# lpylpy0514/VitTracker

Measured on AMD Instinct MI355X. Metric: track() frames/sec per GPU, vit_48_h32, 128px search / 64px template, higher is better.
Workload: dtype f32

## Files before the change

vittracker_amd/csrc/vittrack.hip:

```cpp
#include "../../include/vittrack.h"

#include <hip/hip_runtime.h>

#include <algorithm>
#include <array>
#include <cmath>
#include <cstdio>
#include <cstdlib>
#include <cstring>
#include <map>
#include <mutex>
#include <string>
#include <utility>
#include <vector>

#include "vb_api.h"
#include "vt_blocks.h"
#include "vt_blocks_tile.h"
#include "vt_head.h"
#ifndef VT_SEQ3_MAXP
#define VT_SEQ3_MAXP 2
#endif
#include "vt_head3.h"
#include "vt_generic.h"
// ... 133 lines not shown
    VbModel* vb = nullptr;
    bool generic = false;
    vtg::Dims gd{48, 1, 32};
    DevBuf g_stem_w[4], g_stem_b[4];
    DevBuf g_blocks;
    DevBuf g_head;
    DevBuf g_a, g_b;
    DevBuf g_qkv, g_ao, g_hid, g_x;
    vt_config cfg{};
    Switches sw;
    int len_z = 0, len_x = 0, L = 0, F = 0, Fz = 0;
    bool weights_loaded = false;
    DevBuf stem_w[4], stem_b[4];
    DevBuf stem_w3b;
    DevBuf stem_w4b;
    DevBuf stem_w2k;
    DevBuf stem_w1u;
    std::vector<double> stem_w1_f64, stem_b1_f64;
    float norm_mean[3] = {0.485f, 0.456f, 0.406f}, norm_std[3] = {0.229f, 0.224f, 0.225f};
    DevBuf pos_z, pos_x;
    DevBuf blocks;
    DevBuf blocks3;
    DevBuf head;
    DevBuf head3;
    DevBuf window;
    DevBuf act_x, act_z;
    DevBuf tokens, feat;
    DevBuf tokens_c;
    DevBuf tile_q, tile_k, tile_v, tile_x;
    DevBuf head_m1;
    int head_m1_frames = 0;
// ... 378 lines not shown
    if (m->generic) {
        if (xu8 && zmode != 1) return fail(VT_ERR_STATE, "this stem form has no uint8-patch variant");
        return gen_stem(m, z, x, B, st, tokens, zmode, xu8);
    }
    StemForm f;
    if (int rc = select_stem(m, form_b(m, B), zmode, xu8, &f)) return rc;
    const float* const w1 = xu8 ? m->stem_w1u.p : m->stem_w[0].p;
    const float* const b1 = xu8 ? m->stem_w1u.p + vts::W1U_BIAS : m->stem_b[0].p;
    const int Tx = m->cfg.search_size, Tz = m->cfg.template_size;
    float* const act_x = m->act_x.p + f0 * (size_t)(Tx / 4) * (Tx / 4) * 12;
    float* const act_z = m->act_z.p + f0 * (size_t)(Tz / 4) * (Tz / 4) * 12;
    const int skip_a = m->sw.skip_stem_a;
#ifndef VT_F16
    if (f.stream) {
        hipLaunchKernelGGL(f.stream->k, dim3(B), dim3(f.stream->block), f.stream->lds, st, z, x, w1, b1, m->stem_b[1].p, m->stem_w[2].p, m->stem_b[2].p,
                           m->stem_w[3].p, m->stem_b[3].p, m->pos_z.p, m->pos_x.p, tokens, m->L, m->len_z, m->stem_w2k.p);
        HIP_TRY(hipGetLastError());
        return VT_OK;
    }
#endif
    if (f.fused) {
        hipLaunchKernelGGL(f.fused->k, dim3(B), dim3(f.fused->block), f.fused->lds, st, z, x, w1, b1, m->stem_w[1].p, m->stem_b[1].p, m->stem_w[2].p,
                           m->stem_b[2].p, m->stem_w[3].p, m->stem_b[3].p, m->pos_z.p, m->pos_x.p, tokens, m->L, m->len_z, skip_a, m->dbg_stamps,
                           m->stem_w2k.p, m->stem_w3b.p, m->stem_w4b.p);
        HIP_TRY(hipGetLastError());
        return VT_OK;
    }
    vts::CropA ax{x, act_x, Tx, f.px.r2, zmode == 2 ? 0 : (Tx / 4) / f.px.r2}, az{z, act_z, Tz, f.pz.r2, zmode == 1 ? 0 : (Tz / 4) / f.pz.r2};
    if (f.pipe)
        hipLaunchKernelGGL(f.pipe->k, dim3(B), dim3(f.pipe->block), f.pipe->lds, st, z, x, w1, b1, m->stem_w[1].p, m->stem_b[1].p, act_z, act_x, skip_a,
                           m->dbg_stamps, m->stem_w2k.p);
    else if (f.a2)
        hipLaunchKernelGGL(vts::stem_a2_kernel, dim3(B * ax.bands), dim3(256), f.lds_a, st, ax, az, m->stem_w[0].p, m->stem_b[0].p, m->stem_w[1].p,
                           m->stem_b[1].p, skip_a);
    else
        hipLaunchKernelGGL(f.a->k, dim3(B * (ax.bands + az.bands)), dim3(f.a->block), f.lds_a, st, ax, az, w1, b1, m->stem_w[1].p, m->stem_b[1].p, skip_a);
    HIP_TRY(hipGetLastError());
    vts::CropB bx{act_x, m->pos_x.p, Tx / 4, f.px.r4, zmode == 2 ? 0 : (Tx / 16) / f.px.r4, m->len_z};
    vts::CropB bz{act_z, m->pos_z.p, Tz / 4, f.pz.r4, zmode == 1 ? 0 : (Tz / 16) / f.pz.r4, 0};
    hipLaunchKernelGGL(f.b->k, dim3(B * (bx.bands + bz.bands)), dim3(f.b->block), f.lds_b, st, bx, bz, m->stem_w[2].p, m->stem_b[2].p, m->stem_w[3].p,
                       m->stem_b[3].p, tokens, m->L, m->sw.skip_stem_b);
    HIP_TRY(hipGetLastError());
    return VT_OK;
}

struct BlocksForm {
// ... 548 lines not shown
    }
    if (rc) {
        vt_destroy(m);
        return rc;
    }
    *out = m;
    return VT_OK;
}

void vt_destroy(vt_model* m) {
    if (!m) return;
    for (vt_graph* g : m->graphs) g->owner = nullptr;
    m->graphs.clear();
    if (m->vb) vb::destroy(m->vb);
    for (int i = 0; i < 4; ++i) { m->stem_w[i].release(); m->stem_b[i].release(); }
    m->stem_w2k.release();
    m->stem_w1u.release();
    m->stem_w3b.release();
    m->stem_w4b.release();
    m->act_x.release(); m->act_z.release();
    DevBuf* all[] = {&m->pos_z, &m->pos_x, &m->blocks, &m->blocks3, &m->head, &m->head3, &m->window, &m->tokens, &m->feat, &m->zcache, &m->zstage, &m->imsizes, &m->vlscr, &m->tokens_c,
                     &m->tile_q, &m->tile_k, &m->tile_v, &m->tile_x, &m->head_m1,
                     &m->score, &m->size, &m->offset, &m->pred, &m->hann, &m->conf};
    for (DevBuf* d : all) d->release();
    for (int i = 0; i < 4; ++i) { m->g_stem_w[i].release(); m->g_stem_b[i].release(); }
    DevBuf* gen[] = {&m->g_blocks, &m->g_head, &m->g_a, &m->g_b, &m->g_qkv, &m->g_ao, &m->g_hid, &m->g_x};
    for (DevBuf* d : gen) d->release();
    if (m->cap_stream) (void)hipStreamDestroy(m->cap_stream);
    for (int i = 0; i < 3; ++i) {
        if (m->side_stream[i]) (void)hipStreamDestroy(m->side_stream[i]);
        if (m->join_ev[i]) (void)hipEventDestroy(m->join_ev[i]);
// ... 492 lines not shown
```

vittracker_amd/csrc/vt_conv.h:

```cpp
#pragma once
#include "vt_common.h"

namespace vtc {

template <int NQ>
__device__ __forceinline__ void decode_quad(int Q, int& tap, int& icq) {
    constexpr int NQT = 9 * NQ;
    Q = Q < NQT ? Q : NQT - 1;
    tap = Q / NQ;
    icq = Q - tap * NQ;
}

template <int NOT, int MAXC, int NCH>
__device__ __forceinline__ void load_weights(const float* __restrict__ wimg, int c0, int n, int lane,
                                             opnd (&a)[MAXC][NOT]) {
#pragma unroll
    for (int k = 0; k < MAXC; ++k)
        if (k < n)
#pragma unroll
            for (int ot = 0; ot < NOT; ++ot) a[k][ot] = *reinterpret_cast<const opnd*>(wimg + ((size_t)(ot * NCH + c0 + k) * 64 + lane) * 4);
    __builtin_amdgcn_sched_barrier(0);
}
template <int NOT, int MAXC, int NCH>
__device__ __forceinline__ void load_weights_f4(const float* __restrict__ wimg, int c0, int n, int lane,
// ... 54 lines not shown
                                                f4 (&acc)[NPT][NOT]) {
    constexpr int FULL = NCH / MAXC, REM = NCH % MAXC;
#pragma unroll
    for (int p = 0; p < FULL; ++p) {
        opnd a[MAXC][NOT];
        load_weights<NOT, MAXC, NCH>(wimg, p * MAXC, MAXC, lane, a);
        mma_pass<NOT, NPT, MAXC, MAXC>(in_map, base, a, p * MAXC, off, acc);
    }
    if constexpr (REM > 0) {
        opnd a[MAXC][NOT];
        load_weights<NOT, MAXC, NCH>(wimg, FULL * MAXC, REM, lane, a);
        mma_pass<NOT, NPT, MAXC, REM>(in_map, base, a, FULL * MAXC, off, acc);
    }
}

}
```

vittracker_amd/csrc/vt_head3.h:

```cpp
#pragma once
#include "vt_bf3.h"
#include "vt_head.h"

#ifndef VT_F16
#ifndef VT_SEQ3_C2_MAXP
#define VT_SEQ3_C2_MAXP 5
#endif
#ifndef VT_SEQ3_C2_ACT
#define VT_SEQ3_C2_ACT 8
#endif
#ifndef VT_H3_SKIP
#define VT_H3_SKIP 0
#endif
namespace vth3 {

using vth::C;
using vth::W1;
using vth::nchunks;
using vth::ntiles;
using vt3::bf16x8;
using vt3::u32x2;
using vt3::u32x4;
using vt3::split3;
using vt3::join3;
// ... 155 lines not shown
                    acc = __builtin_amdgcn_mfma_f32_16x16x32_bf16(__builtin_bit_cast(bf16x8, ww[wp]), __builtin_bit_cast(bf16x8, x[xp]), acc, 0, 0, 0);
                };
                if (!(VT_H3_SKIP & 2)) { mm(2, 0); mm(0, 2); mm(1, 1); mm(1, 0); mm(0, 1); mm(0, 0); }
            }
            if (p == NSP - 1 && 4 * q < COUT) {
                f4 v = acc;
                v.x = fmaxf(v.x, 0.f); v.y = fmaxf(v.y, 0.f); v.z = fmaxf(v.z, 0.f); v.w = fmaxf(v.w, 0.f);
                out_map[q * G::NPIX + centre] = v;
            }
            pipe.park(g + 1);
            __syncthreads();
        }
    }
};

template <int AB>
__device__ __forceinline__ f4 mfma4x4_bcast(float a, float b, f4 c) { return __builtin_amdgcn_mfma_f32_4x4x1f32(a, b, c, 4, AB, 0); }
__device__ __forceinline__ f4 mfma4x4_bcast(float a, float b, f4 c, int ab) {
    switch (ab) {
        case 0: return mfma4x4_bcast<0>(a, b, c);   case 1: return mfma4x4_bcast<1>(a, b, c);
        case 2: return mfma4x4_bcast<2>(a, b, c);   case 3: return mfma4x4_bcast<3>(a, b, c);
        case 4: return mfma4x4_bcast<4>(a, b, c);   case 5: return mfma4x4_bcast<5>(a, b, c);
        case 6: return mfma4x4_bcast<6>(a, b, c);   case 7: return mfma4x4_bcast<7>(a, b, c);
        case 8: return mfma4x4_bcast<8>(a, b, c);   case 9: return mfma4x4_bcast<9>(a, b, c);
        case 10: return mfma4x4_bcast<10>(a, b, c); case 11: return mfma4x4_bcast<11>(a, b, c);
        case 12: return mfma4x4_bcast<12>(a, b, c); case 13: return mfma4x4_bcast<13>(a, b, c);
        case 14: return mfma4x4_bcast<14>(a, b, c); default: return mfma4x4_bcast<15>(a, b, c);
    }
}
constexpr int quad_nkr(int nq) { return (9 * nq * 4 + 15) / 16; }
template <int NQ, int PLANE, typename Off>
__device__ __forceinline__ void quad_taps(const f4* in0, Off off, const float (&wr)[quad_nkr(NQ)], f4 (&acc)[4]) {
    f4 bv[2][NQ];
    auto fetch = [&](int tap, f4 (&bd)[NQ]) {
        const int o = off(tap);
#pragma unroll
        for (int icq = 0; icq < NQ; ++icq) bd[icq] = in0[icq * PLANE + o];
        __builtin_amdgcn_sched_barrier(0);
    };
    fetch(0, bv[0]);
#pragma unroll
    for (int tap = 0; tap < 9; ++tap) {
        if (tap + 1 < 9) fetch(tap + 1, bv[(tap + 1) & 1]);
#pragma unroll
// ... 519 lines not shown
```

vittracker_amd/csrc/vt_stem.h:

```cpp
#pragma once
#include <type_traits>

#include "vt_common.h"
#include "vt_conv.h"

namespace vts {

typedef __attribute__((address_space(4))) const float* sptr;
__device__ __forceinline__ sptr opaque(const float* p) {
    unsigned long long v = reinterpret_cast<unsigned long long>(p);
    asm volatile("" : "+s"(v));
    return (sptr)v;
}

constexpr int round16(int v) { return (v + 15) & ~15; }
template <int NQ>
__device__ __forceinline__ int s2_chunk_off(int c, int q, int npix_in, int pitch_in, int half_in) {
    int tap, icq;
    vtc::decode_quad<NQ>(4 * c + q, tap, icq);
    const int dy = tap / 3, dx = tap - 3 * dy;
    return icq * npix_in + dy * pitch_in + (dx == 1 ? 0 : (dx == 0 ? half_in : half_in + 1));
}

__device__ __forceinline__ int ilog2(int v) { return 31 - __clz(v); }
// ... 71 lines not shown
}
template <bool ZERO_TOP, typename Band>
__device__ __forceinline__ void ring_edges(f4* ring, const f4* other_ring, int pair, const Band& J, bool halo) {
    const int nrow = 2 * J.R2 + 1;
    if (pair < 2 * nrow) {
        const int plane = pair >= nrow ? 1 : 0;
        ring[plane * J.npix1 + (pair - plane * nrow) * J.PITCH + J.HALF] = splat4(0.f);
    }
    if ((ZERO_TOP || halo) && pair >= 128 && pair < 128 + 2 * J.PITCH) {
        const int e = pair - 128, plane = e >= J.PITCH ? 1 : 0, col = e - plane * J.PITCH;
        ring[plane * J.npix1 + col] = halo ? other_ring[plane * J.npix1 + 2 * J.R2 * J.PITCH + col] : splat4(0.f);
    }
}

#ifndef VT_F16
typedef float f16v __attribute__((ext_vector_type(16)));
template <typename Band>
__device__ __forceinline__ f16v l2_tile4(const f4* ring, const Band& J, const f4* cw2, const float* cb2, int gw, int q, int px) {
    const int op = 16 * (4 * gw + q) + px, yy = op >> J.lgW2, xx = op & ((1 << J.lgW2) - 1);
    const f4* src = ring + 2 * yy * J.PITCH + xx;
    const f4* wk = cw2 + px;
    const f4 bv2 = ld4(cb2 + 4 * q);
    f16v acc = {bv2.x, bv2.y, bv2.z, bv2.w, bv2.x, bv2.y, bv2.z, bv2.w, bv2.x, bv2.y, bv2.z, bv2.w, bv2.x, bv2.y, bv2.z, bv2.w};
    auto tapoff = [&](int tap) {
        const int dy = tap / 3, dx = tap - 3 * dy;
        return dy * J.PITCH + (dx == 1 ? 0 : (dx == 0 ? J.HALF : J.HALF + 1));
    };
    f4 a0 = src[tapoff(0)], a1 = src[J.npix1 + tapoff(0)], w0 = wk[0], w1 = wk[16];
#pragma unroll
    for (int tap = 0; tap < 9; ++tap) {
        f4 na0 = a0, na1 = a1, nw0 = w0, nw1 = w1;
        if (tap + 1 < 9) {
            na0 = src[tapoff(tap + 1)]; na1 = src[J.npix1 + tapoff(tap + 1)];
            nw0 = wk[32 * (tap + 1)]; nw1 = wk[32 * (tap + 1) + 16];
            __builtin_amdgcn_sched_barrier(0);
        }
        acc = __builtin_amdgcn_mfma_f32_16x16x1f32(w0.x, a0.x, acc, 0, 0, 0);
        acc = __builtin_amdgcn_mfma_f32_16x16x1f32(w0.y, a0.y, acc, 0, 0, 0);
        acc = __builtin_amdgcn_mfma_f32_16x16x1f32(w0.z, a0.z, acc, 0, 0, 0);
        acc = __builtin_amdgcn_mfma_f32_16x16x1f32(w0.w, a0.w, acc, 0, 0, 0);
        acc = __builtin_amdgcn_mfma_f32_16x16x1f32(w1.x, a1.x, acc, 0, 0, 0);
        acc = __builtin_amdgcn_mfma_f32_16x16x1f32(w1.y, a1.y, acc, 0, 0, 0);
        a0 = na0; a1 = na1; w0 = nw0; w1 = nw1;
    }
    return acc;
}
__device__ __forceinline__ f4 l2_result(const f16v& acc, int bb) {
    return hardswish4(f4{acc[4 * bb], acc[4 * bb + 1], acc[4 * bb + 2], acc[4 * bb + 3]});
}
#else
template <typename Band, typename Store>
__device__ __forceinline__ void l2_tiles_f16(const f4* ring, const Band& J, const f4* cw2, const float* cb2, int lane, int gw, int q, int px, Store store) {
    f4 w2a[5][1];
#pragma unroll
    for (int c = 0; c < 5; ++c) w2a[c][0] = cw2[c * 64 + lane];
    const f4 bv2 = ld4(cb2 + 4 * q);
    int base[2], yy[2], xx[2];
#pragma unroll
    for (int i = 0; i < 2; ++i) {
        const int op = 16 * (gw + 8 * i) + px;
        yy[i] = op >> J.lgW2; xx[i] = op & ((1 << J.lgW2) - 1);
        base[i] = 2 * yy[i] * J.PITCH + xx[i];
    }
// ... 445 lines not shown
```

vittracker_amd/csrc/vt_stem_fused.h:

```cpp
#pragma once
#include <type_traits>

#include "vt_common.h"
#include "vt_bf3.h"
#include "vt_conv.h"
#include "vt_stem.h"

namespace vts {

template <bool DIAG>
__device__ __forceinline__ void stamp_wave(unsigned long long* stamps, int b, int wave, int lane, int& nstamp) {
    if constexpr (DIAG) {
        if (stamps != nullptr && nstamp < 32) {
            unsigned long long tt;
            asm volatile("s_memtime %0\n\ts_waitcnt lgkmcnt(0)" : "=s"(tt)::"memory");
            if (lane == 0) stamps[((size_t)b * 16 + wave) * 32 + nstamp] = tt;
            ++nstamp;
        }
    }
}

struct FusedGeo {
    static constexpr int TX = 128, TZ = 64;
    static constexpr int R2X = 8, NBX = (TX / 4) / R2X;
// ... 32 lines not shown
    static constexpr int npix1 = IS_Z ? G::NPIX1Z : G::NPIX1X;
    static constexpr int R2 = IS_Z ? G::R2Z : G::R2X, p0 = IS_Z ? 0 : XB * G::R2X, lgW2 = lgT - 2;
    static constexpr int m2_off = IS_Z ? 3 * G::NPIX2X : 0, pitch2 = (T >> 2) + 1, half2 = T >> 3;
    static constexpr int npix2 = IS_Z ? G::NPIX2Z : G::NPIX2X;
    static constexpr bool halo = !IS_Z && XB > 0;
    const float* in;
};

template <int ZMODE, bool DIAG, bool L3B = true, bool U8 = false>
__global__ __launch_bounds__(1024) void stem_fused_kernel(
    const float* __restrict__ zin, const float* __restrict__ xin,
    const float* __restrict__ w1g, const float* __restrict__ b1, const float* __restrict__ w2img, const float* __restrict__ b2,
    const float* __restrict__ w3img, const float* __restrict__ b3, const float* __restrict__ w4img, const float* __restrict__ b4,
    const float* __restrict__ pos_z, const float* __restrict__ pos_x, float* __restrict__ tokens, int L, int len_z, int skip_arg,
    unsigned long long* __restrict__ stamps,
    const float* __restrict__ w2k,
    const float* __restrict__ w3b,
    const float* __restrict__ w4b) {
    using G = FusedGeo;
    static_assert(!U8 || ZMODE == 1, "the uint8 patch form is the search-only (cached template) step");
    constexpr bool L3BF3 = L3B && !VT_IS_F16;
    constexpr bool do_z = ZMODE != 1, do_x = ZMODE != 2;
    const int skip = DIAG ? skip_arg : 0;
    extern __shared__ __attribute__((aligned(16))) float lds_f[];
    f4* const lds = reinterpret_cast<f4*>(lds_f);
    f4* const ring0 = lds;
    f4* const m2 = lds + 2 * G::RING;
    constexpr int M2Z_OFF = 3 * G::NPIX2X;
    f4* const m3x = lds;
    f4* const m3z = lds + 6 * G::NPIX3X;
    vt3::u32x2* const m3xp = reinterpret_cast<vt3::u32x2*>(lds);
// ... 67 lines not shown
        }
#pragma unroll
        for (int j = 0; j < 6; ++j) { a0[j] = hardswish(a0[j]); a1[j] = hardswish(a1[j]); }
        f4* dst = ring + lr * J.PITCH;
        dst[qp] = f4{a0[0], a0[1], a0[2], a0[3]};
        dst[J.npix1 + qp] = f4{a0[4], a0[5], 0.f, 0.f};
        dst[J.HALF + 1 + qp] = f4{a1[0], a1[1], a1[2], a1[3]};
        dst[J.npix1 + J.HALF + 1 + qp] = f4{a1[4], a1[5], 0.f, 0.f};
        __builtin_amdgcn_s_setprio(0);
    };

    auto layer2 = [&](const auto& J) {
#ifndef VT_F16
        if (gw < 4) {
            const int ln = fresh(lane), q = ln >> 4, px = ln & 15;
            const f16v acc = l2_tile4(ring, J, cw2, cb2, gw, q, px);
            if (q < 3) {
#pragma unroll
                for (int bb = 0; bb < 4; ++bb) {
                    const int ob = 16 * (4 * gw + bb) + px, y = ob >> J.lgW2, x = ob & ((1 << J.lgW2) - 1);
                    m2[J.m2_off + q * J.npix2 + (J.p0 + y + 1) * J.pitch2 + ((x & 1) ? J.half2 + 1 + (x >> 1) : (x >> 1))] = l2_result(acc, bb);
                }
            }
        }
#else
        l2_tiles_f16(ring, J, cw2, cb2, lane, gw, q, px, [&](int y, int x, f4 v) {
            m2[J.m2_off + q * J.npix2 + (J.p0 + y + 1) * J.pitch2 + ((x & 1) ? J.half2 + 1 + (x >> 1) : (x >> 1))] = v;
        });
#endif
    };

    int nstamp = 0;
    auto stamp = [&]() { stamp_wave<DIAG>(stamps, b, wave, lane, nstamp); };
    stamp();
    L1In<U8> v;
    const int t = threadIdx.x;
#ifndef VT_F16
    constexpr int NW2 = 9 * 32;
    const float* const w2src = w2k;
#else
    constexpr int NW2 = 5 * 64;
    const float* const w2src = w2img;
#endif
    const float* csrc = w2src;
    const bool has_c = t < NW2 || (t >= 320 && t < 344);
    if (t < NW2) csrc = w2src + 4 * t;
    else if (t >= 320 && t < 324) csrc = b2 + 4 * (t - 320);
    else if (t >= 324 && t < 332) csrc = b3 + 4 * (t - 324);
    else if (t >= 332 && t < 344) csrc = b4 + 4 * (t - 332);
    const f4 cst = ld4(csrc);
    __builtin_amdgcn_sched_barrier(0);
#ifndef VT_SF_STAGGER
#define VT_SF_STAGGER 6
#endif
// ... 296 lines not shown
struct PipeGeo {
    static constexpr int R2X = band_r2(TX), R2Z = band_r2(TZ);
    static constexpr int NBX = (TX / 4) / R2X, NBZ = (TZ / 4) / R2Z, NB = NBX + NBZ;
    static constexpr int RING = 2 * (band_npix1(TX) > band_npix1(TZ) ? band_npix1(TX) : band_npix1(TZ));
    static constexpr int CONST_F4 = 5 * 64 + 4;
    static constexpr int LDS_BYTES = (2 * RING + CONST_F4) * 16;
    static_assert(NB % 2 == 0 && NBZ % 2 == 0, "bands alternate between the two groups, crop by crop");
    static_assert((R2X * (TX / 4)) == 256 && (R2Z * (TZ / 4)) == 256, "16 layer-2 tiles per band");
};

template <int TX, int TZ, int ZMODE, bool DIAG, bool U8 = false>
__global__ __launch_bounds__(1024) void stem_pipe_kernel(
    const float* __restrict__ zin, const float* __restrict__ xin, const float* __restrict__ w1g, const float* __restrict__ b1,
    const float* __restrict__ w2img, const float* __restrict__ b2, float* __restrict__ act_z, float* __restrict__ act_x, int skip_arg,
    unsigned long long* __restrict__ stamps,
    const float* __restrict__ w2k) {
    using G = PipeGeo<TX, TZ>;
    static_assert(!U8 || ZMODE == 1, "the uint8 patch form is the search-only (cached template) step");
    const int skip = DIAG ? skip_arg : 0;
    constexpr int s_lo = ZMODE == 1 ? G::NBZ / 2 : 0, s_hi = ZMODE == 2 ? G::NBZ / 2 : G::NB / 2;
    extern __shared__ __attribute__((aligned(16))) float lds_f[];
    f4* const ring0 = reinterpret_cast<f4*>(lds_f);
    f4* const cw2 = ring0 + 2 * G::RING;
    const float* const cb2 = reinterpret_cast<const float*>(cw2 + 5 * 64);

    const int b = blockIdx.x;
    const int lane = threadIdx.x & 63;
    const int wave = __builtin_amdgcn_readfirstlane(threadIdx.x >> 6);
    const int grp = wave >> 3, gw = wave & 7;
    const int q = lane >> 4, px = lane & 15;
    f4* const ring = ring0 + grp * G::RING;
// ... 58 lines not shown
                    a1[j] = fmaf(t1[s], cur[s * 6 + j], a1[j]);
                }
        }
#pragma unroll
        for (int j = 0; j < 6; ++j) { a0[j] = hardswish(a0[j]); a1[j] = hardswish(a1[j]); }
        f4* dst = ring + lr * J.PITCH;
        dst[qp] = f4{a0[0], a0[1], a0[2], a0[3]};
        dst[J.npix1 + qp] = f4{a0[4], a0[5], 0.f, 0.f};
        dst[J.HALF + 1 + qp] = f4{a1[0], a1[1], a1[2], a1[3]};
        dst[J.npix1 + J.HALF + 1 + qp] = f4{a1[4], a1[5], 0.f, 0.f};
        __builtin_amdgcn_s_setprio(0);
    };
    auto layer2 = [&](const Band& J) {
#ifndef VT_F16
        if (gw < 4) {
            const f16v acc = l2_tile4(ring, J, cw2, cb2, gw, q, px);
            if (q < 3) {
#pragma unroll
                for (int bb = 0; bb < 4; ++bb) {
                    const int ob = 16 * (4 * gw + bb) + px, y = ob >> J.lgW2, x = ob & ((1 << J.lgW2) - 1);
                    st4(J.out + ((((size_t)q << (2 * J.lgW2)) + (((size_t)J.p0 + y) << J.lgW2) + x) << 2), l2_result(acc, bb));
                }
            }
        }
#else
        l2_tiles_f16(ring, J, cw2, cb2, lane, gw, q, px, [&](int y, int x, f4 v) {
            st4(J.out + ((((size_t)q << (2 * J.lgW2)) + (((size_t)J.p0 + y) << J.lgW2) + x) << 2), v);
        });
#endif
    };

    int nstamp = 0;
    auto stamp = [&]() { stamp_wave<DIAG>(stamps, b, wave, lane, nstamp); };
    stamp();
    L1In<U8> v;
    fetch(band(2 * s_lo + grp), v);
#ifndef VT_F16
    if (threadIdx.x < 9 * 32) cw2[threadIdx.x] = ld4(w2k + 4 * threadIdx.x);
#else
    if (threadIdx.x < 5 * 64) cw2[threadIdx.x] = ld4(w2img + 4 * threadIdx.x);
#endif
    else if (threadIdx.x < 5 * 64) {}
    else if (threadIdx.x < 5 * 64 + 4) cw2[threadIdx.x] = ld4(b2 + 4 * (threadIdx.x - 320));
    if (grp == 1) __syncthreads();
    for (int s = s_lo; s < s_hi; ++s) {
        const int j = 2 * s + grp;
        if (!(skip & 1)) layer1(band(j), v);
        stamp();
        __syncthreads();
        stamp();
        fetch(band(j + 2 < 2 * s_hi ? j + 2 : j), v);
        if (!(skip & 2)) layer2(band(j));
        stamp();
// ... 8 lines not shown
```

vittracker_amd/csrc/vt_stem_stream.h:

```cpp
#pragma once
#include "vt_common.h"
#include "vt_conv.h"
#include "vt_stem.h"

#ifndef VT_F16
#ifndef VT_SS_PRIO34
#define VT_SS_PRIO34 2
#endif
#ifndef VT_SS_PRIO2
#define VT_SS_PRIO2 0
#endif
#ifndef VT_SS_SKIP
#define VT_SS_SKIP 0
#endif
namespace vts {

template <int TX, int TZ>
struct StreamGeo {
    static constexpr int NBX = (TX / 4) / band_r2(TX), NBZ = (TZ / 4) / band_r2(TZ), NB = NBX + NBZ;
    static constexpr int np2(int T) { return round16((band_r2(T) + 1) * (T / 4 + 1)); }
    static constexpr int np3(int T) { return round16((band_r2(T) / 2 + 1) * (T / 8 + 1)); }
    static constexpr int imax(int a, int b) { return a > b ? a : b; }
    static constexpr int RING = 2 * imax(band_npix1(TX), band_npix1(TZ));
    static constexpr int SLOT2 = 3 * imax(np2(TX), np2(TZ));
    static constexpr int SLOT3 = 6 * imax(np3(TX), np3(TZ));
    static constexpr int CONST_F4 = 9 * 32 + 4 + 8 + 12;
    static constexpr int OFF3 = 8, OFF4 = 16;
    static constexpr int OFFTAB_F4 = (2 * 4 * OFF3 + 2 * 4 * OFF4) / 8;
    static constexpr int W4L_F4 = 3 * 64;
    static constexpr int LDS_F4 = 2 * RING + 3 * SLOT2 + 3 * SLOT3 + CONST_F4 + OFFTAB_F4 + W4L_F4;
    static constexpr int LDS_BYTES = LDS_F4 * 16;
    static_assert(LDS_BYTES <= 160 * 1024, "LDS");
    static_assert(band_r2(TX) % 4 == 0 && band_r2(TZ) % 4 == 0, "a band holds whole token rows");
};

template <int TX, int TZ, int ZMODE, bool U8 = false>
__global__ __launch_bounds__(1024) void stem_stream_kernel(
    const float* __restrict__ zin, const float* __restrict__ xin,
    const float* __restrict__ w1g, const float* __restrict__ b1, const float* __restrict__ b2, const float* __restrict__ w3img,
    const float* __restrict__ b3, const float* __restrict__ w4img, const float* __restrict__ b4, const float* __restrict__ pos_z,
    const float* __restrict__ pos_x, float* __restrict__ tokens, int L, int len_z,
    const float* __restrict__ w2k) {
    using G = StreamGeo<TX, TZ>;
    static_assert(!U8 || ZMODE == 1, "the uint8 patch form is the search-only (cached template) step");
    constexpr int g_lo = ZMODE == 1 ? G::NBZ : 0, g_hi = ZMODE == 2 ? G::NBZ : G::NB;
    constexpr int NIV = g_hi - g_lo + 3, NIV2 = (NIV + 1) / 2;
    extern __shared__ __attribute__((aligned(16))) float lds_f[];
    f4* const lds = reinterpret_cast<f4*>(lds_f);
    f4* const ring0 = lds;
    f4* const l2ring = lds + 2 * G::RING;
    f4* const l3ring = l2ring + 3 * G::SLOT2;
    f4* const cw2 = l3ring + 3 * G::SLOT3;
    const float* const cb2 = reinterpret_cast<const float*>(cw2 + 9 * 32);
    const float* const cb3 = cb2 + 16;
    const float* const cb4 = cb3 + 32;
    int* const otab = reinterpret_cast<int*>(cw2 + G::CONST_F4);
    f4* const w4l = cw2 + G::CONST_F4 + G::OFFTAB_F4;

    const int b = blockIdx.x;
    const int lane = threadIdx.x & 63;
    const int wave = __builtin_amdgcn_readfirstlane(threadIdx.x >> 6);
    auto fresh = [](int v) { asm volatile("" : "+v"(v)); return v; };

    struct Band {
        bool is_z;
        int kb, nb;
        int lgT, HALF, lgHALF, PITCH, npix1, R2, lgW2;
        int pitch2, half2, np2;
// ... 6 lines not shown
        static_assert((1 << lgTX) == TX && (1 << lgTZ) == TZ, "crop sides");
        J.is_z = g < G::NBZ;
        J.kb = J.is_z ? g : g - G::NBZ;
        J.nb = J.is_z ? G::NBZ : G::NBX;
        const int T = J.is_z ? TZ : TX;
        J.lgT = J.is_z ? lgTZ : lgTX; J.HALF = T >> 2; J.lgHALF = J.lgT - 2; J.PITCH = (T >> 1) + 1;
        J.npix1 = J.is_z ? band_npix1(TZ) : band_npix1(TX); J.R2 = J.is_z ? band_r2(TZ) : band_r2(TX); J.lgW2 = J.lgT - 2;
        J.pitch2 = (T >> 2) + 1; J.half2 = T >> 3; J.np2 = J.is_z ? G::np2(TZ) : G::np2(TX);
        J.lgW3 = J.lgT - 3; J.R3 = J.R2 >> 1; J.pitch3 = (T >> 3) + 1; J.half3 = T >> 4; J.np3 = J.is_z ? G::np3(TZ) : G::np3(TX);
        J.lgW4 = J.lgT - 4;
        return J;
    };

    {
        const int t = threadIdx.x;
        if (t < 9 * 32) cw2[t] = ld4(w2k + 4 * t);
        else if (t < 9 * 32 + 4) cw2[t] = ld4(b2 + 4 * (t - 288));
        else if (t < 9 * 32 + 12) cw2[t] = ld4(b3 + 4 * (t - 292));
        else if (t < 9 * 32 + 24) cw2[t] = ld4(b4 + 4 * (t - 300));
        else if (t >= 320 && t < 320 + 4 * G::OFFTAB_F4) {
            const int e0 = t - 320;
            const bool l4 = e0 >= 4 * G::OFF3;
            const int e = l4 ? e0 - 4 * G::OFF3 : e0, per = l4 ? 2 * G::OFF4 : 2 * G::OFF3;
            const bool isz = e >= per;
            const int r = isz ? e - per : e, rowi = l4 ? G::OFF4 / 2 : G::OFF3 / 2, qq = r / rowi, c = 2 * (r - qq * rowi);
            const int T = isz ? TZ : TX;
            int v[2];
#pragma unroll
            for (int h = 0; h < 2; ++h)
                v[h] = l4 ? s2_chunk_off<6>(c + h, qq, isz ? G::np3(TZ) : G::np3(TX), (T >> 3) + 1, T >> 4)
                          : s2_chunk_off<3>(c + h, qq, isz ? G::np2(TZ) : G::np2(TX), (T >> 2) + 1, T >> 3);
            otab[e0] = v[0] | (v[1] << 16);
        }
    }
// ... 68 lines not shown
        const int gw = wave - 8;
        auto layer2 = [&](const Band& J, int g) {
            const int ln = fresh(lane), q = ln >> 4, px = ln & 15, tid2 = gw * 64 + ln;
            const f4* const ring = ring0 + (g & 1) * G::RING;
            f4* const slot = l2ring + (g % 3) * G::SLOT2;
            f4* const nslot = l2ring + ((g + 1) % 3) * G::SLOT2;
            if (tid2 < 3 * (J.R2 + 1)) {
                const int plane = tid2 / (J.R2 + 1), row = tid2 - plane * (J.R2 + 1);
                slot[plane * J.np2 + row * J.pitch2 + J.half2] = splat4(0.f);
            }
            if (J.kb == 0)
                for (int e = tid2; e < 3 * J.pitch2; e += 256) {
                    const int plane = e / J.pitch2, col = e - plane * J.pitch2;
                    slot[plane * J.np2 + col] = splat4(0.f);
                }
            const f16v acc = l2_tile4(ring, J, cw2, cb2, gw, q, px);
            if (q < 3) {
                const bool copy_down = J.kb + 1 < J.nb;
#pragma unroll
                for (int bb = 0; bb < 4; ++bb) {
                    const int ob = 16 * (4 * gw + bb) + px, y = ob >> J.lgW2, x = ob & ((1 << J.lgW2) - 1);
                    const f4 r = l2_result(acc, bb);
                    const int col = (x & 1) ? J.half2 + 1 + (x >> 1) : (x >> 1);
                    slot[q * J.np2 + (y + 1) * J.pitch2 + col] = r;
                    if (copy_down && y == J.R2 - 1) nslot[q * J.np2 + col] = r;
                }
            }
        };
        if (VT_SS_PRIO2 > 0) __builtin_amdgcn_s_setprio(VT_SS_PRIO2);
        __syncthreads();
#pragma unroll 1
        for (int it = 0; it < NIV2; ++it) {
            const int j = g_lo + 2 * it;
            if (j - 1 >= g_lo && j - 1 < g_hi && !(VT_SS_SKIP & 2)) layer2(band(j - 1), j - 1);
            __syncthreads();
            if (j >= g_lo && j < g_hi && !(VT_SS_SKIP & 2)) layer2(band(j), j);
            __syncthreads();
        }
    } else {
        const int w4 = wave - 12;
        constexpr int NCH3 = 7, NCH4 = 14;
// ... 107 lines not shown
```

vittracker_amd/csrc/vt_weights.h:

```cpp
#pragma once

namespace {

using TensorMap = std::map<std::string, std::pair<const float*, int64_t>>;

int need(const TensorMap& tm, const std::string& name, int64_t numel, const float** out) {
    auto it = tm.find(name);
    if (it == tm.end()) return fail(VT_ERR_MISSING_KEY, "missing key in state dict: " + name);
    if (it->second.second != numel)
        return fail(VT_ERR_MISSING_KEY, "shape mismatch for " + name + ": got " + std::to_string(it->second.second) +
                                            " elements, want " + std::to_string(numel));
    *out = it->second.first;
    return VT_OK;
}

int fold_conv_bn(const TensorMap& tm, const std::string& conv, const std::string& bn, bool conv_bias, int cout,
                 int cin, std::vector<double>& w, std::vector<double>& b) {
    const float *pw, *pb = nullptr, *g, *beta, *mu, *var;
    int rc;
    if ((rc = need(tm, conv + ".weight", (int64_t)cout * cin * 9, &pw))) return rc;
    if (conv_bias && (rc = need(tm, conv + ".bias", cout, &pb))) return rc;
    if ((rc = need(tm, bn + ".weight", cout, &g))) return rc;
    if ((rc = need(tm, bn + ".bias", cout, &beta))) return rc;
    if ((rc = need(tm, bn + ".running_mean", cout, &mu))) return rc;
// ... 276 lines not shown
            if ((rc = upload(m->stem_b[i], std::vector<float>(b.begin(), b.end())))) return rc;
            m->stem_w1_f64 = w;
            m->stem_b1_f64 = b;
            if ((rc = fold_w1u(m, m->norm_mean, m->norm_std))) return rc;
        } else {
            const int tiles = (STEM_CH[i + 1] + 15) / 16, nch = (9 * ((STEM_CH[i] + 3) / 4) + 3) / 4;
            std::vector<float> img((size_t)tiles * nch * 256), bias((size_t)tiles * 16, 0.f);
            pack_conv_image(w, STEM_CH[i + 1], STEM_CH[i], img.data());
            for (int o = 0; o < STEM_CH[i + 1]; ++o) bias[o] = (float)b[o];
            if ((rc = upload(m->stem_w[i], img))) return rc;
            if ((rc = upload(m->stem_b[i], bias))) return rc;
#ifdef VT_F16
            if (i >= 2 && (rc = opnd_inplace(m->stem_w[i].p, img.size()))) return rc;
#endif
            if (i == 1) {
                std::vector<float> k((size_t)9 * 2 * 16 * 4, 0.f);
                for (int tap = 0; tap < 9; ++tap)
                    for (int oc = 0; oc < STEM_CH[2]; ++oc)
                        for (int ic = 0; ic < STEM_CH[1]; ++ic)
                            k[(((size_t)tap * 2 + ic / 4) * 16 + oc) * 4 + ic % 4] = (float)w[((size_t)oc * STEM_CH[1] + ic) * 9 + tap];
                if ((rc = upload(m->stem_w2k, k))) return rc;
            }
            if (i == 2) {
                std::vector<uint16_t> img3((size_t)2 * 4 * 3 * 64 * 8, 0);
                pack_conv_image3(w, STEM_CH[3], STEM_CH[2], img3.data());
                std::vector<float> as_f(img3.size() / 2);
                std::memcpy(as_f.data(), img3.data(), img3.size() * 2);
                if ((rc = upload(m->stem_w3b, as_f))) return rc;
            }
            if (i == 3) {
                std::vector<uint16_t> img4((size_t)3 * 7 * 3 * 64 * 8, 0);
                pack_conv_image3(w, STEM_CH[4], STEM_CH[3], img4.data());
                std::vector<float> as_f(img4.size() / 2);
                std::memcpy(as_f.data(), img4.data(), img4.size() * 2);
                if ((rc = upload(m->stem_w4b, as_f))) return rc;
            }
// ... 123 lines not shown
```

Measured before the change: 3.206 million.

## Recast stem layer-2 conv as broadcast 4x4x1 MFMAs over three output quads

Replaces the layer-2 stem conv's 16x16x1 MFMA tile (16 output channels, 12 used, 54 MFMAs with wasted lanes) with 4x4x1 MFMAs that broadcast one lane's weight per k-step across three 4-channel groups. Weights are repacked so each lane holds its k-slice in registers, and each 16-lane block handles one pixel row group. The aim is to stop computing the 4 padding output channels and to cut weight traffic from LDS, which shrinks the constant weight area. The trade-off is more MFMA issues (162 of the 4x4 variant) and a switch-based broadcast selector.

Result: no change. 3.227 million, median of 6 (+0.7%).

```diff
diff --git a/vittracker_amd/csrc/vittrack.hip b/vittracker_amd/csrc/vittrack.hip
--- a/vittracker_amd/csrc/vittrack.hip
+++ b/vittracker_amd/csrc/vittrack.hip
@@ -171,7 +171,7 @@
     DevBuf stem_w[4], stem_b[4];
     DevBuf stem_w3b;
     DevBuf stem_w4b;
-    DevBuf stem_w2k;
+    DevBuf stem_w2q;
     DevBuf stem_w1u;
     std::vector<double> stem_w1_f64, stem_b1_f64;
     float norm_mean[3] = {0.485f, 0.456f, 0.406f}, norm_std[3] = {0.229f, 0.224f, 0.225f};
@@ -580,7 +580,7 @@
 #ifndef VT_F16
     if (f.stream) {
         hipLaunchKernelGGL(f.stream->k, dim3(B), dim3(f.stream->block), f.stream->lds, st, z, x, w1, b1, m->stem_b[1].p, m->stem_w[2].p, m->stem_b[2].p,
-                           m->stem_w[3].p, m->stem_b[3].p, m->pos_z.p, m->pos_x.p, tokens, m->L, m->len_z, m->stem_w2k.p);
+                           m->stem_w[3].p, m->stem_b[3].p, m->pos_z.p, m->pos_x.p, tokens, m->L, m->len_z, m->stem_w2q.p);
         HIP_TRY(hipGetLastError());
         return VT_OK;
     }
@@ -588,14 +588,14 @@
     if (f.fused) {
         hipLaunchKernelGGL(f.fused->k, dim3(B), dim3(f.fused->block), f.fused->lds, st, z, x, w1, b1, m->stem_w[1].p, m->stem_b[1].p, m->stem_w[2].p,
                            m->stem_b[2].p, m->stem_w[3].p, m->stem_b[3].p, m->pos_z.p, m->pos_x.p, tokens, m->L, m->len_z, skip_a, m->dbg_stamps,
-                           m->stem_w2k.p, m->stem_w3b.p, m->stem_w4b.p);
+                           m->stem_w2q.p, m->stem_w3b.p, m->stem_w4b.p);
         HIP_TRY(hipGetLastError());
         return VT_OK;
     }
     vts::CropA ax{x, act_x, Tx, f.px.r2, zmode == 2 ? 0 : (Tx / 4) / f.px.r2}, az{z, act_z, Tz, f.pz.r2, zmode == 1 ? 0 : (Tz / 4) / f.pz.r2};
     if (f.pipe)
         hipLaunchKernelGGL(f.pipe->k, dim3(B), dim3(f.pipe->block), f.pipe->lds, st, z, x, w1, b1, m->stem_w[1].p, m->stem_b[1].p, act_z, act_x, skip_a,
-                           m->dbg_stamps, m->stem_w2k.p);
+                           m->dbg_stamps, m->stem_w2q.p);
     else if (f.a2)
         hipLaunchKernelGGL(vts::stem_a2_kernel, dim3(B * ax.bands), dim3(256), f.lds_a, st, ax, az, m->stem_w[0].p, m->stem_b[0].p, m->stem_w[1].p,
                            m->stem_b[1].p, skip_a);
@@ -1174,7 +1174,7 @@
     m->graphs.clear();
     if (m->vb) vb::destroy(m->vb);
     for (int i = 0; i < 4; ++i) { m->stem_w[i].release(); m->stem_b[i].release(); }
-    m->stem_w2k.release();
+    m->stem_w2q.release();
     m->stem_w1u.release();
     m->stem_w3b.release();
     m->stem_w4b.release();
diff --git a/vittracker_amd/csrc/vt_conv.h b/vittracker_amd/csrc/vt_conv.h
--- a/vittracker_amd/csrc/vt_conv.h
+++ b/vittracker_amd/csrc/vt_conv.h
@@ -92,4 +92,19 @@
     }
 }
 
+template <int AB>
+__device__ __forceinline__ f4 mfma4x4_bcast(float a, float b, f4 c) { return __builtin_amdgcn_mfma_f32_4x4x1f32(a, b, c, 4, AB, 0); }
+__device__ __forceinline__ f4 mfma4x4_bcast(float a, float b, f4 c, int ab) {
+    switch (ab) {
+        case 0: return mfma4x4_bcast<0>(a, b, c);   case 1: return mfma4x4_bcast<1>(a, b, c);
+        case 2: return mfma4x4_bcast<2>(a, b, c);   case 3: return mfma4x4_bcast<3>(a, b, c);
+        case 4: return mfma4x4_bcast<4>(a, b, c);   case 5: return mfma4x4_bcast<5>(a, b, c);
+        case 6: return mfma4x4_bcast<6>(a, b, c);   case 7: return mfma4x4_bcast<7>(a, b, c);
+        case 8: return mfma4x4_bcast<8>(a, b, c);   case 9: return mfma4x4_bcast<9>(a, b, c);
+        case 10: return mfma4x4_bcast<10>(a, b, c); case 11: return mfma4x4_bcast<11>(a, b, c);
+        case 12: return mfma4x4_bcast<12>(a, b, c); case 13: return mfma4x4_bcast<13>(a, b, c);
+        case 14: return mfma4x4_bcast<14>(a, b, c); default: return mfma4x4_bcast<15>(a, b, c);
+    }
 }
+
+}
diff --git a/vittracker_amd/csrc/vt_head3.h b/vittracker_amd/csrc/vt_head3.h
--- a/vittracker_amd/csrc/vt_head3.h
+++ b/vittracker_amd/csrc/vt_head3.h
@@ -193,20 +193,7 @@
     }
 };
 
-template <int AB>
-__device__ __forceinline__ f4 mfma4x4_bcast(float a, float b, f4 c) { return __builtin_amdgcn_mfma_f32_4x4x1f32(a, b, c, 4, AB, 0); }
-__device__ __forceinline__ f4 mfma4x4_bcast(float a, float b, f4 c, int ab) {
-    switch (ab) {
-        case 0: return mfma4x4_bcast<0>(a, b, c);   case 1: return mfma4x4_bcast<1>(a, b, c);
-        case 2: return mfma4x4_bcast<2>(a, b, c);   case 3: return mfma4x4_bcast<3>(a, b, c);
-        case 4: return mfma4x4_bcast<4>(a, b, c);   case 5: return mfma4x4_bcast<5>(a, b, c);
-        case 6: return mfma4x4_bcast<6>(a, b, c);   case 7: return mfma4x4_bcast<7>(a, b, c);
-        case 8: return mfma4x4_bcast<8>(a, b, c);   case 9: return mfma4x4_bcast<9>(a, b, c);
-        case 10: return mfma4x4_bcast<10>(a, b, c); case 11: return mfma4x4_bcast<11>(a, b, c);
-        case 12: return mfma4x4_bcast<12>(a, b, c); case 13: return mfma4x4_bcast<13>(a, b, c);
-        case 14: return mfma4x4_bcast<14>(a, b, c); default: return mfma4x4_bcast<15>(a, b, c);
-    }
-}
+using vtc::mfma4x4_bcast;
 constexpr int quad_nkr(int nq) { return (9 * nq * 4 + 15) / 16; }
 template <int NQ, int PLANE, typename Off>
 __device__ __forceinline__ void quad_taps(const f4* in0, Off off, const float (&wr)[quad_nkr(NQ)], f4 (&acc)[4]) {
diff --git a/vittracker_amd/csrc/vt_stem.h b/vittracker_amd/csrc/vt_stem.h
--- a/vittracker_amd/csrc/vt_stem.h
+++ b/vittracker_amd/csrc/vt_stem.h
@@ -109,39 +109,42 @@
 }
 
 #ifndef VT_F16
-typedef float f16v __attribute__((ext_vector_type(16)));
+constexpr int L2Q_F4 = 3 * 4 * 64 / 4;
 template <typename Band>
-__device__ __forceinline__ f16v l2_tile4(const f4* ring, const Band& J, const f4* cw2, const float* cb2, int gw, int q, int px) {
-    const int op = 16 * (4 * gw + q) + px, yy = op >> J.lgW2, xx = op & ((1 << J.lgW2) - 1);
+__device__ __forceinline__ void l2_quads(const f4* ring, const Band& J, const f4* cw2, const float* cb2, int gw, int b, int px, f4 (&acc)[3]) {
+    const int op = 16 * (4 * gw + b) + px, yy = op >> J.lgW2, xx = op & ((1 << J.lgW2) - 1);
     const f4* src = ring + 2 * yy * J.PITCH + xx;
-    const f4* wk = cw2 + px;
-    const f4 bv2 = ld4(cb2 + 4 * q);
-    f16v acc = {bv2.x, bv2.y, bv2.z, bv2.w, bv2.x, bv2.y, bv2.z, bv2.w, bv2.x, bv2.y, bv2.z, bv2.w, bv2.x, bv2.y, bv2.z, bv2.w};
+    const float* wl = reinterpret_cast<const float*>(cw2) + 16 * b + px;
     auto tapoff = [&](int tap) {
         const int dy = tap / 3, dx = tap - 3 * dy;
         return dy * J.PITCH + (dx == 1 ? 0 : (dx == 0 ? J.HALF : J.HALF + 1));
     };
-    f4 a0 = src[tapoff(0)], a1 = src[J.npix1 + tapoff(0)], w0 = wk[0], w1 = wk[16];
+    float wr[3][4];
+#pragma unroll
+    for (int g = 0; g < 3; ++g) wr[g][0] = wl[(4 * g) * 64];
+    f4 a0 = src[tapoff(0)], a1 = src[J.npix1 + tapoff(0)];
+#pragma unroll
+    for (int g = 0; g < 3; ++g)
+#pragma unroll
+        for (int kg = 1; kg < 4; ++kg) wr[g][kg] = wl[(4 * g + kg) * 64];
+#pragma unroll
+    for (int g = 0; g < 3; ++g) acc[g] = ld4(cb2 + 4 * g);
 #pragma unroll
     for (int tap = 0; tap < 9; ++tap) {
-        f4 na0 = a0, na1 = a1, nw0 = w0, nw1 = w1;
+        f4 na0 = a0, na1 = a1;
         if (tap + 1 < 9) {
             na0 = src[tapoff(tap + 1)]; na1 = src[J.npix1 + tapoff(tap + 1)];
-            nw0 = wk[32 * (tap + 1)]; nw1 = wk[32 * (tap + 1) + 16];
             __builtin_amdgcn_sched_barrier(0);
         }
-        acc = __builtin_amdgcn_mfma_f32_16x16x1f32(w0.x, a0.x, acc, 0, 0, 0);
-        acc = __builtin_amdgcn_mfma_f32_16x16x1f32(w0.y, a0.y, acc, 0, 0, 0);
-        acc = __builtin_amdgcn_mfma_f32_16x16x1f32(w0.z, a0.z, acc, 0, 0, 0);
-        acc = __builtin_amdgcn_mfma_f32_16x16x1f32(w0.w, a0.w, acc, 0, 0, 0);
-        acc = __builtin_amdgcn_mfma_f32_16x16x1f32(w1.x, a1.x, acc, 0, 0, 0);
-        acc = __builtin_amdgcn_mfma_f32_16x16x1f32(w1.y, a1.y, acc, 0, 0, 0);
-        a0 = na0; a1 = na1; w0 = nw0; w1 = nw1;
-    }
-    return acc;
-}
-__device__ __forceinline__ f4 l2_result(const f16v& acc, int bb) {
-    return hardswish4(f4{acc[4 * bb], acc[4 * bb + 1], acc[4 * bb + 2], acc[4 * bb + 3]});
+#pragma unroll
+        for (int ic = 0; ic < 6; ++ic) {
+            const int k = 6 * tap + ic;
+            const float av = ic < 4 ? a0[ic] : a1[ic - 4];
+#pragma unroll
+            for (int g = 0; g < 3; ++g) acc[g] = vtc::mfma4x4_bcast(wr[g][k >> 4], av, acc[g], k & 15);
+        }
+        a0 = na0; a1 = na1;
+    }
 }
 #else
 template <typename Band, typename Store>
diff --git a/vittracker_amd/csrc/vt_stem_fused.h b/vittracker_amd/csrc/vt_stem_fused.h
--- a/vittracker_amd/csrc/vt_stem_fused.h
+++ b/vittracker_amd/csrc/vt_stem_fused.h
@@ -70,7 +70,7 @@
     const float* __restrict__ w3img, const float* __restrict__ b3, const float* __restrict__ w4img, const float* __restrict__ b4,
     const float* __restrict__ pos_z, const float* __restrict__ pos_x, float* __restrict__ tokens, int L, int len_z, int skip_arg,
     unsigned long long* __restrict__ stamps,
-    const float* __restrict__ w2k,
+    const float* __restrict__ w2q,
     const float* __restrict__ w3b,
     const float* __restrict__ w4b) {
     using G = FusedGeo;
@@ -168,14 +168,12 @@
 #ifndef VT_F16
         if (gw < 4) {
             const int ln = fresh(lane), q = ln >> 4, px = ln & 15;
-            const f16v acc = l2_tile4(ring, J, cw2, cb2, gw, q, px);
-            if (q < 3) {
-#pragma unroll
-                for (int bb = 0; bb < 4; ++bb) {
-                    const int ob = 16 * (4 * gw + bb) + px, y = ob >> J.lgW2, x = ob & ((1 << J.lgW2) - 1);
-                    m2[J.m2_off + q * J.npix2 + (J.p0 + y + 1) * J.pitch2 + ((x & 1) ? J.half2 + 1 + (x >> 1) : (x >> 1))] = l2_result(acc, bb);
-                }
-            }
+            f4 acc[3];
+            l2_quads(ring, J, cw2, cb2, gw, q, px, acc);
+            const int ob = 16 * (4 * gw + q) + px, y = ob >> J.lgW2, x = ob & ((1 << J.lgW2) - 1);
+            f4* const dst = m2 + J.m2_off + (J.p0 + y + 1) * J.pitch2 + ((x & 1) ? J.half2 + 1 + (x >> 1) : (x >> 1));
+#pragma unroll
+            for (int g = 0; g < 3; ++g) dst[g * J.npix2] = hardswish4(acc[g]);
         }
 #else
         l2_tiles_f16(ring, J, cw2, cb2, lane, gw, q, px, [&](int y, int x, f4 v) {
@@ -190,8 +188,8 @@
     L1In<U8> v;
     const int t = threadIdx.x;
 #ifndef VT_F16
-    constexpr int NW2 = 9 * 32;
-    const float* const w2src = w2k;
+    constexpr int NW2 = L2Q_F4;
+    const float* const w2src = w2q;
 #else
     constexpr int NW2 = 5 * 64;
     const float* const w2src = w2img;
@@ -518,7 +516,7 @@
     const float* __restrict__ zin, const float* __restrict__ xin, const float* __restrict__ w1g, const float* __restrict__ b1,
     const float* __restrict__ w2img, const float* __restrict__ b2, float* __restrict__ act_z, float* __restrict__ act_x, int skip_arg,
     unsigned long long* __restrict__ stamps,
-    const float* __restrict__ w2k) {
+    const float* __restrict__ w2q) {
     using G = PipeGeo<TX, TZ>;
     static_assert(!U8 || ZMODE == 1, "the uint8 patch form is the search-only (cached template) step");
     const int skip = DIAG ? skip_arg : 0;
@@ -607,14 +605,12 @@
     auto layer2 = [&](const Band& J) {
 #ifndef VT_F16
         if (gw < 4) {
-            const f16v acc = l2_tile4(ring, J, cw2, cb2, gw, q, px);
-            if (q < 3) {
-#pragma unroll
-                for (int bb = 0; bb < 4; ++bb) {
-                    const int ob = 16 * (4 * gw + bb) + px, y = ob >> J.lgW2, x = ob & ((1 << J.lgW2) - 1);
-                    st4(J.out + ((((size_t)q << (2 * J.lgW2)) + (((size_t)J.p0 + y) << J.lgW2) + x) << 2), l2_result(acc, bb));
-                }
-            }
+            f4 acc[3];
+            l2_quads(ring, J, cw2, cb2, gw, q, px, acc);
+            const int ob = 16 * (4 * gw + q) + px, y = ob >> J.lgW2, x = ob & ((1 << J.lgW2) - 1);
+#pragma unroll
+            for (int g = 0; g < 3; ++g)
+                st4(J.out + ((((size_t)g << (2 * J.lgW2)) + (((size_t)J.p0 + y) << J.lgW2) + x) << 2), hardswish4(acc[g]));
         }
 #else
         l2_tiles_f16(ring, J, cw2, cb2, lane, gw, q, px, [&](int y, int x, f4 v) {
@@ -629,7 +625,7 @@
     L1In<U8> v;
     fetch(band(2 * s_lo + grp), v);
 #ifndef VT_F16
-    if (threadIdx.x < 9 * 32) cw2[threadIdx.x] = ld4(w2k + 4 * threadIdx.x);
+    if (threadIdx.x < L2Q_F4) cw2[threadIdx.x] = ld4(w2q + 4 * threadIdx.x);
 #else
     if (threadIdx.x < 5 * 64) cw2[threadIdx.x] = ld4(w2img + 4 * threadIdx.x);
 #endif
diff --git a/vittracker_amd/csrc/vt_stem_stream.h b/vittracker_amd/csrc/vt_stem_stream.h
--- a/vittracker_amd/csrc/vt_stem_stream.h
+++ b/vittracker_amd/csrc/vt_stem_stream.h
@@ -24,7 +24,7 @@
     static constexpr int RING = 2 * imax(band_npix1(TX), band_npix1(TZ));
     static constexpr int SLOT2 = 3 * imax(np2(TX), np2(TZ));
     static constexpr int SLOT3 = 6 * imax(np3(TX), np3(TZ));
-    static constexpr int CONST_F4 = 9 * 32 + 4 + 8 + 12;
+    static constexpr int CONST_F4 = L2Q_F4 + 4 + 8 + 12;
     static constexpr int OFF3 = 8, OFF4 = 16;
     static constexpr int OFFTAB_F4 = (2 * 4 * OFF3 + 2 * 4 * OFF4) / 8;
     static constexpr int W4L_F4 = 3 * 64;
@@ -40,7 +40,7 @@
     const float* __restrict__ w1g, const float* __restrict__ b1, const float* __restrict__ b2, const float* __restrict__ w3img,
     const float* __restrict__ b3, const float* __restrict__ w4img, const float* __restrict__ b4, const float* __restrict__ pos_z,
     const float* __restrict__ pos_x, float* __restrict__ tokens, int L, int len_z,
-    const float* __restrict__ w2k) {
+    const float* __restrict__ w2q) {
     using G = StreamGeo<TX, TZ>;
     static_assert(!U8 || ZMODE == 1, "the uint8 patch form is the search-only (cached template) step");
     constexpr int g_lo = ZMODE == 1 ? G::NBZ : 0, g_hi = ZMODE == 2 ? G::NBZ : G::NB;
@@ -51,7 +51,7 @@
     f4* const l2ring = lds + 2 * G::RING;
     f4* const l3ring = l2ring + 3 * G::SLOT2;
     f4* const cw2 = l3ring + 3 * G::SLOT3;
-    const float* const cb2 = reinterpret_cast<const float*>(cw2 + 9 * 32);
+    const float* const cb2 = reinterpret_cast<const float*>(cw2 + L2Q_F4);
     const float* const cb3 = cb2 + 16;
     const float* const cb4 = cb3 + 32;
     int* const otab = reinterpret_cast<int*>(cw2 + G::CONST_F4);
@@ -88,10 +88,10 @@
 
     {
         const int t = threadIdx.x;
-        if (t < 9 * 32) cw2[t] = ld4(w2k + 4 * t);
-        else if (t < 9 * 32 + 4) cw2[t] = ld4(b2 + 4 * (t - 288));
-        else if (t < 9 * 32 + 12) cw2[t] = ld4(b3 + 4 * (t - 292));
-        else if (t < 9 * 32 + 24) cw2[t] = ld4(b4 + 4 * (t - 300));
+        if (t < L2Q_F4) cw2[t] = ld4(w2q + 4 * t);
+        else if (t < L2Q_F4 + 4) cw2[t] = ld4(b2 + 4 * (t - L2Q_F4));
+        else if (t < L2Q_F4 + 12) cw2[t] = ld4(b3 + 4 * (t - L2Q_F4 - 4));
+        else if (t < L2Q_F4 + 24) cw2[t] = ld4(b4 + 4 * (t - L2Q_F4 - 12));
         else if (t >= 320 && t < 320 + 4 * G::OFFTAB_F4) {
             const int e0 = t - 320;
             const bool l4 = e0 >= 4 * G::OFF3;
@@ -190,17 +190,16 @@
                     const int plane = e / J.pitch2, col = e - plane * J.pitch2;
                     slot[plane * J.np2 + col] = splat4(0.f);
                 }
-            const f16v acc = l2_tile4(ring, J, cw2, cb2, gw, q, px);
-            if (q < 3) {
-                const bool copy_down = J.kb + 1 < J.nb;
-#pragma unroll
-                for (int bb = 0; bb < 4; ++bb) {
-                    const int ob = 16 * (4 * gw + bb) + px, y = ob >> J.lgW2, x = ob & ((1 << J.lgW2) - 1);
-                    const f4 r = l2_result(acc, bb);
-                    const int col = (x & 1) ? J.half2 + 1 + (x >> 1) : (x >> 1);
-                    slot[q * J.np2 + (y + 1) * J.pitch2 + col] = r;
-                    if (copy_down && y == J.R2 - 1) nslot[q * J.np2 + col] = r;
-                }
+            f4 acc[3];
+            l2_quads(ring, J, cw2, cb2, gw, q, px, acc);
+            const bool copy_down = J.kb + 1 < J.nb;
+            const int ob = 16 * (4 * gw + q) + px, y = ob >> J.lgW2, x = ob & ((1 << J.lgW2) - 1);
+            const int col = (x & 1) ? J.half2 + 1 + (x >> 1) : (x >> 1);
+#pragma unroll
+            for (int g = 0; g < 3; ++g) {
+                const f4 r = hardswish4(acc[g]);
+                slot[g * J.np2 + (y + 1) * J.pitch2 + col] = r;
+                if (copy_down && y == J.R2 - 1) nslot[g * J.np2 + col] = r;
             }
         };
         if (VT_SS_PRIO2 > 0) __builtin_amdgcn_s_setprio(VT_SS_PRIO2);
diff --git a/vittracker_amd/csrc/vt_weights.h b/vittracker_amd/csrc/vt_weights.h
--- a/vittracker_amd/csrc/vt_weights.h
+++ b/vittracker_amd/csrc/vt_weights.h
@@ -314,12 +314,15 @@
             if (i >= 2 && (rc = opnd_inplace(m->stem_w[i].p, img.size()))) return rc;
 #endif
             if (i == 1) {
-                std::vector<float> k((size_t)9 * 2 * 16 * 4, 0.f);
-                for (int tap = 0; tap < 9; ++tap)
-                    for (int oc = 0; oc < STEM_CH[2]; ++oc)
-                        for (int ic = 0; ic < STEM_CH[1]; ++ic)
-                            k[(((size_t)tap * 2 + ic / 4) * 16 + oc) * 4 + ic % 4] = (float)w[((size_t)oc * STEM_CH[1] + ic) * 9 + tap];
-                if ((rc = upload(m->stem_w2k, k))) return rc;
+                static_assert(STEM_CH[2] == 12 && STEM_CH[1] == 6, "l2_quads: three groups of four output channels over 54 k-steps");
+                std::vector<float> k((size_t)3 * 4 * 64, 0.f);
+                for (int g = 0; g < 3; ++g)
+                    for (int kg = 0; kg < 4; ++kg)
+                        for (int l = 0; l < 64; ++l) {
+                            const int kk = 16 * kg + (l >> 2), tap = kk / 6, ic = kk % 6, oc = 4 * g + (l & 3);
+                            if (kk < 54) k[((size_t)g * 4 + kg) * 64 + l] = (float)w[((size_t)oc * STEM_CH[1] + ic) * 9 + tap];
+                        }
+                if ((rc = upload(m->stem_w2q, k))) return rc;
             }
             if (i == 2) {
                 std::vector<uint16_t> img3((size_t)2 * 4 * 3 * 64 * 8, 0);
```
